# shangfuu/avse_challenge

Measured on AMD Instinct MI355X. Metric: utterances/sec (3s@16kHz + 75 lip frames), higher is better.
Workload: dtype fp32; 1 GPU; avse1 AV baseline train step (BASELINE configs[1]): HIP STFT front-end + AVNet (ResNet18 lip enc + TCN, dilated Conv2d audio net, LSTM fusion) fwd/bwd + Adam; global_batch=32, per_gpu_batch=32, seq_len=48000, stft_frames=376, lip_frames=75, lip_hw=96, parallelism=dp1, hip_graph=fwd+bwd+opt

## Files before the change

avse_challenge_amd/csrc/dconv.hip:

```cpp
#include <algorithm>

#include "bnact_cols.h"
#include "common.h"

namespace avse {
namespace dcf {

typedef _Float16 half8 __attribute__((ext_vector_type(8)));
typedef float floatx16 __attribute__((ext_vector_type(16)));
typedef int i4_t __attribute__((ext_vector_type(4)));
typedef __attribute__((address_space(3))) void lds_void_t;

constexpr int C = 64, KS = 5, NQ = 4, TP = 256, THREADS = 256, WAVES = THREADS / 64;
constexpr int ROWB = 64;
constexpr int WIMG = KS * C * ROWB;
constexpr int NSTG = KS * NQ;
constexpr int MAXD = 16;
constexpr int XIMG_MAX = (TP + 8 * MAXD) * ROWB;
constexpr int STAGE = XIMG_MAX + WIMG;
constexpr int NBUF = 3;
constexpr int MAXP = (XIMG_MAX + WIMG) / 1024 / WAVES + 1;
static_assert(NBUF * STAGE <= 160 * 1024, "LDS");

__device__ inline int swz(int r) { return (r >> 2) & 3; }

__device__ inline int split_exp(uint32_t mb) {
    const int ef = (int)((mb >> 23) & 0xff);
    if (mb == 0) return 0;
    const int k = ef == 0 ? -127 : ef - 127;
    return min(100, max(-100, 14 - k));
}

__device__ inline i4_t rsrc_of(const void* base, int64_t bytes) {
    if (bytes > 0x7FFFFFF0LL) bytes = 0x7FFFFFF0LL;
    const uint64_t a = (uint64_t)base;
    return i4_t{__builtin_amdgcn_readfirstlane((int)(uint32_t)a), __builtin_amdgcn_readfirstlane((int)((a >> 32) & 0xffff)),
                __builtin_amdgcn_readfirstlane((int)bytes), 0x00020000};
}

__device__ inline void dma16(i4_t r, uint32_t lds_addr, uint32_t voff) {
    asm volatile("s_mov_b32 m0, %2\n\tbuffer_load_dwordx4 %0, %1, 0 offen lds" ::"v"(voff), "s"(r), "s"(lds_addr)
                 : "memory");
}

__device__ inline uint32_t lds_u32(const void* p) {
    return __builtin_amdgcn_readfirstlane((uint32_t)(uintptr_t)(const lds_void_t*)p);
}

__device__ inline void wait_all_but(int n) {
    switch (n) {
        case 0: asm volatile("s_waitcnt vmcnt(0)" ::: "memory"); break;
        case 1: asm volatile("s_waitcnt vmcnt(1)" ::: "memory"); break;
        case 2: asm volatile("s_waitcnt vmcnt(2)" ::: "memory"); break;
        case 3: asm volatile("s_waitcnt vmcnt(3)" ::: "memory"); break;
        case 4: asm volatile("s_waitcnt vmcnt(4)" ::: "memory"); break;
        case 5: asm volatile("s_waitcnt vmcnt(5)" ::: "memory"); break;
        case 6: asm volatile("s_waitcnt vmcnt(6)" ::: "memory"); break;
        case 7: asm volatile("s_waitcnt vmcnt(7)" ::: "memory"); break;
        case 8: asm volatile("s_waitcnt vmcnt(8)" ::: "memory"); break;
        case 9: asm volatile("s_waitcnt vmcnt(9)" ::: "memory"); break;
        case 10: asm volatile("s_waitcnt vmcnt(10)" ::: "memory"); break;
        case 11: asm volatile("s_waitcnt vmcnt(11)" ::: "memory"); break;
        default: asm volatile("s_waitcnt vmcnt(12)" ::: "memory"); break;
    }
}

__device__ inline half8 frag(const uint8_t* img, int row, int c) {
    return *reinterpret_cast<const half8*>(img + row * ROWB + 16 * (c ^ swz(row)));
}

struct Args {
    const void* xq;
    const void* wq;
    const uint32_t* maxbits;
    const float* bias;
    float* y;
    int N, H, W, tiles;
    bnact::BnEpi bn;
};

template <int D, int NW, int WGS = 1, int EPI = 0>
__global__ __launch_bounds__(64 * NW, WGS) void fwd_kernel(Args a) {
    constexpr int TPX = 64 * NW, NSEG = NW == 4 ? 2 : 3;
    constexpr int NP = (TPX + 4 * D * NSEG + 15) / 16 * 16;
    constexpr int XIMG = NP * ROWB;
    constexpr int STG = XIMG + WIMG;
    constexpr int NB = WGS == 2 ? 2 : ((3 * STG <= 160 * 1024) ? 3 : 2);
    constexpr int PX = XIMG / 1024, PT = PX + WIMG / 1024;
    constexpr int MP = PT / NW + 1;
    __shared__ __attribute__((aligned(1024))) uint8_t lds[NB * STG];
    const int lane = threadIdx.x & 63;
    const int wave = __builtin_amdgcn_readfirstlane(threadIdx.x >> 6);
    const int bid = xcd_remap(blockIdx.x, gridDim.x);
    const int n = bid / a.tiles, t = bid % a.tiles;
    const int HW = a.H * a.W;
    const int p0 = t * TPX;
    const int r0 = p0 / a.W, w0 = p0 - r0 * a.W;
    const int n0 = min(TPX, a.W - w0), n1 = min(TPX - n0, a.W), n2 = TPX - n0 - n1;
    const int S1 = n0 + 4 * D, S2 = n0 + n1 + 8 * D;
    const i4_t rx = rsrc_of(a.xq, (int64_t)a.N * HW * 256);
    const i4_t rw = rsrc_of(a.wq, (int64_t)NSTG * WIMG);
    const uint32_t lds0 = lds_u32(lds);

    int pcol[MP], prow[MP];
    uint32_t pchunk[MP];
    const int npieces = (PT - wave + NW - 1) / NW;
#pragma unroll
    for (int m = 0; m < MP; ++m) {
        const int k = wave + NW * m;
        if (k < PX) {
            const int r = 16 * k + (lane >> 2), c = (lane & 3) ^ swz(r);
            int col, row;
            if (r < S1) {
                col = w0 - 2 * D + r;
                row = r0;
            } else if (r < S2 || NSEG == 2) {
                col = -2 * D + (r - S1);
                row = (n1 > 0 && r < S1 + n1 + 4 * D) ? r0 + 1 : -1000000;
            } else {
                col = -2 * D + (r - S2);
                row = (n2 > 0 && r < S2 + n2 + 4 * D) ? r0 + 2 : -1000000;
            }
            pcol[m] = (col >= 0 && col < a.W) ? col : -1;
            prow[m] = row;
            pchunk[m] = 16u * c;
        } else {
            const int r = 16 * (k - PX) + (lane >> 2), c = (lane & 3) ^ swz(r);
            pcol[m] = 0;
            prow[m] = 0;
            pchunk[m] = (uint32_t)(r * ROWB + 16 * c);
        }
    }
    auto issue = [&](int s) {
        const int kh = s / NQ, q = s % NQ;
        const uint32_t img = lds0 + (s % NB) * STG;
#pragma unroll
        for (int m = 0; m < MP; ++m) {
            if (m >= npieces) break;
            const int k = wave + NW * m;
            if (k < PX) {
                const int row = prow[m] + D * (kh - 2);
                const bool ok = pcol[m] >= 0 && row >= 0 && row < a.H;
                const uint32_t pix = ((uint32_t)n * (uint32_t)a.H + (uint32_t)row) * (uint32_t)a.W + (uint32_t)pcol[m];
                const uint32_t off = ok ? pix * 256u + (uint32_t)(q * 64) + pchunk[m] : 0x7FFFFFF0u;
                dma16(rx, img + k * 1024, off);
            } else {
                dma16(rw, img + XIMG + (k - PX) * 1024, (uint32_t)(s * WIMG) + pchunk[m]);
            }
        }
    };

    int posA[2];
#pragma unroll
    for (int i = 0; i < 2; ++i) {
        const int j = 64 * wave + 32 * i + (lane & 31);
        posA[i] = j + 4 * D * ((j >= n0) + (j >= n0 + n1));
    }
    const int hc = lane >> 5;

    floatx16 acc[2][2];
#pragma unroll
    for (int i = 0; i < 2; ++i)
#pragma unroll
        for (int j = 0; j < 2; ++j)
#pragma unroll
            for (int e = 0; e < 16; ++e) acc[i][j][e] = 0.f;

    issue(0);
    if (NB == 3) issue(1);
    for (int s = 0; s < NSTG; ++s) {
        if (NB == 3 && s + 1 < NSTG) wait_all_but(npieces);
        else asm volatile("s_waitcnt vmcnt(0)" ::: "memory");
        __builtin_amdgcn_s_barrier();
        asm volatile("" ::: "memory");
        if (s + NB - 1 < NSTG) issue(s + NB - 1);
        const uint8_t* ximg = lds + (s % NB) * STG;
        const uint8_t* wimg = ximg + XIMG;
#pragma unroll
        for (int kw = 0; kw < KS; ++kw) {
            half8 ah[2], al[2], bh[2], bl[2];
#pragma unroll
            for (int i = 0; i < 2; ++i) {
                const int r = posA[i] + D * kw;
                ah[i] = frag(ximg, r, hc);
                al[i] = frag(ximg, r, 2 + hc);
            }
#pragma unroll
            for (int j = 0; j < 2; ++j) {
                const int r = kw * C + 32 * j + (lane & 31);
                bh[j] = frag(wimg, r, hc);
                bl[j] = frag(wimg, r, 2 + hc);
            }
#pragma unroll
            for (int i = 0; i < 2; ++i)
#pragma unroll
                for (int j = 0; j < 2; ++j) {
                    acc[i][j] = __builtin_amdgcn_mfma_f32_32x32x16_f16(ah[i], bh[j], acc[i][j], 0, 0, 0);
                    acc[i][j] = __builtin_amdgcn_mfma_f32_32x32x16_f16(ah[i], bl[j], acc[i][j], 0, 0, 0);
                    acc[i][j] = __builtin_amdgcn_mfma_f32_32x32x16_f16(al[i], bh[j], acc[i][j], 0, 0, 0);
                }
        }
        if (NB == 2) {
            asm volatile("s_waitcnt lgkmcnt(0)" ::: "memory");
        }
    }

    const float scale = __builtin_ldexpf(1.f, -(split_exp(a.maxbits[0]) + split_exp(a.maxbits[1])));
    auto store = [&](int j) {
        const int o = 32 * j + (lane & 31);
        const float bv = a.bias ? a.bias[o] : 0.f;
#pragma unroll
        for (int i = 0; i < 2; ++i)
#pragma unroll
            for (int g = 0; g < 4; ++g)
#pragma unroll
                for (int e = 0; e < 4; ++e) {
                    const int p = p0 + 64 * wave + 32 * i + 8 * g + 4 * (lane >> 5) + e;
                    const float v = acc[i][j][4 * g + e] * scale + bv;
                    if constexpr (EPI != 0) acc[i][j][4 * g + e] = v;
                    if (p < HW) a.y[((int64_t)n * HW + p) * C + o] = v;
                }
    };
    if constexpr (EPI == 0) {
#pragma unroll
        for (int j = 0; j < 2; ++j) store(j);
    } else {
        constexpr int ENQ = EPI == 2 ? 4 : 3;
        float* part = reinterpret_cast<float*>(lds);
        __syncthreads();
        bnact::bn_epi_wave<bnact::ACT_RELU, EPI == 2>(
            a.bn, [&](int i, int j, int r) { return acc[i][j][r]; }, store, (int64_t)n * HW + p0 + 64 * wave,
            (int64_t)(n + 1) * HW, 0, C, lane, part + wave * ENQ * 64);
        __syncthreads();
        bnact::bn_epi_row<EPI == 2>(a.bn, part, NW, 1, (int64_t)bid, 0, C);
    }
}

constexpr int WG_CHUNK = 64;
constexpr int PIXB = 256;
constexpr int WTHREADS = 512, WWAVES = WTHREADS / 64;

typedef short s4_t __attribute__((ext_vector_type(4)));
typedef __attribute__((address_space(3))) s4_t lds_s4_t;

__device__ inline int tswz(int r, int c) { return c ^ (((r & 1) << 1) | ((r & 2) << 2)); }

__device__ inline half8 tfrag(const uint8_t* img, const int (&row)[2], int cb, int pl, int lane) {
    const int g = lane >> 4, i = lane & 15;
    const int q = 2 * cb + (g & 1);
    s4_t v[2];
#pragma unroll
    for (int u = 0; u < 2; ++u) {
        const int r = row[u];
        const int byte = q * 64 + pl * 32 + 8 * (i & 3);
        const int off = r * PIXB + 16 * tswz(r, byte >> 4) + (byte & 15);
        v[u] = __builtin_amdgcn_ds_read_tr16_b64_v4i16((lds_s4_t*)(img + off));
    }
    const s4_t w0 = v[0], w1 = v[1];
    const short __attribute__((ext_vector_type(8))) w = {w0[0], w0[1], w0[2], w0[3], w1[0], w1[1], w1[2], w1[3]};
    return __builtin_bit_cast(half8, w);
}

struct WArgs {
    const void* xq;
    const void* dyq;
    const uint32_t* xmax;
    const uint32_t* dymax;
    float* part;
    float* dbpart;
    int N, H, W, cpi, chunks, ranges;
};

struct ChunkPos {
    int n, p0, hA, wA0;
    __device__ void init(int c, int cpi, int W) {
        n = c / cpi;
        p0 = (c - n * cpi) * WG_CHUNK;
        hA = p0 / W;
        wA0 = p0 - hA * W;
    }
    __device__ void next(int HW, int W) {
        p0 += WG_CHUNK;
        if (p0 >= HW) {
            ++n;
            p0 = hA = wA0 = 0;
        } else {
            wA0 += WG_CHUNK;
            if (wA0 >= W) {
                wA0 -= W;
                ++hA;
            }
        }
    }
};

template <int D>
__global__ __launch_bounds__(WTHREADS, 1) void wgrad_kernel(WArgs a) {
    constexpr int NP = WG_CHUNK + 8 * D;
    constexpr int YIMG = WG_CHUNK * PIXB, XIMG = NP * PIXB, STG = YIMG + XIMG;
    constexpr int NB = (3 * STG <= 160 * 1024) ? 3 : 2;
    constexpr int PY = YIMG / 1024, PT = PY + XIMG / 1024;
    constexpr int MAXPW = PT / WWAVES + 1;
    __shared__ __attribute__((aligned(1024))) uint8_t lds[NB * STG];
    const int lane = threadIdx.x & 63;
    const int wave = __builtin_amdgcn_readfirstlane(threadIdx.x >> 6);
    const int bid = xcd_remap(blockIdx.x, gridDim.x);
    const int r = bid / KS, kh = bid % KS;
    const int c_lo = (int)((int64_t)r * a.chunks / a.ranges), c_hi = (int)((int64_t)(r + 1) * a.chunks / a.ranges);
    const int HW = a.H * a.W;
    const i4_t rx = rsrc_of(a.xq, (int64_t)a.N * HW * PIXB);
    const i4_t ry = rsrc_of(a.dyq, (int64_t)a.N * HW * PIXB);
    const uint32_t lds0 = lds_u32(lds);
    const int npieces = (PT - wave + WWAVES - 1) / WWAVES;
    const int pr = lane >> 4, pc = lane & 15;
    int pj[MAXPW];
    uint32_t psw[MAXPW];
#pragma unroll
    for (int m = 0; m < MAXPW; ++m) {
        const int k = wave + WWAVES * m;
        pj[m] = k < PY ? 4 * k + pr : 4 * (k - PY) + pr;
        psw[m] = 16u * tswz(pj[m], pc);
    }

    auto issue = [&](const ChunkPos& cp, int buf) {
        const int nA = min(WG_CHUNK, a.W - cp.wA0);
        const int row1 = cp.hA + D * (kh - 2), row2 = nA < WG_CHUNK ? row1 + 1 : -1000000;
        const int ybase = cp.n * HW + cp.p0;
        const int nHrow = cp.n * a.H;
        const uint32_t img = lds0 + buf * STG;
#pragma unroll
        for (int m = 0; m < MAXPW; ++m) {
            if (m >= npieces) break;
            const int k = wave + WWAVES * m;
            if (k < PY) {
                const int j = pj[m];
                const uint32_t off = cp.p0 + j < HW ? (uint32_t)(ybase + j) * PIXB + psw[m] : 0x7FFFFFF0u;
                dma16(ry, img + k * 1024, off);
            } else {
                const int q = pj[m];
                const bool s1 = q < nA + 4 * D;
                const int col = s1 ? cp.wA0 - 2 * D + q : q - nA - 6 * D;
                const int row = s1 ? row1 : row2;
                const bool ok = (unsigned)col < (unsigned)a.W && (unsigned)row < (unsigned)a.H;
                const uint32_t pix = (uint32_t)((nHrow + row) * a.W + col);
                dma16(rx, img + YIMG + (k - PY) * 1024, ok ? pix * PIXB + psw[m] : 0x7FFFFFF0u);
            }
        }
    };

    const int half = wave >> 2, ob = (wave >> 1) & 1, ib = wave & 1;
    const bool want_db = a.dbpart != nullptr && kh == 0 && ib == 0;
    floatx16 acc[KS], accb;
#pragma unroll
    for (int k = 0; k < KS; ++k)
#pragma unroll
        for (int e = 0; e < 16; ++e) acc[k][e] = 0.f;
#pragma unroll
    for (int e = 0; e < 16; ++e) accb[e] = 0.f;
    half8 ones;
#pragma unroll
    for (int e = 0; e < 8; ++e) ones[e] = (_Float16)1.0f;

    const int g = lane >> 4, li = lane & 15;
    ChunkPos cc, ci;
    cc.init(c_lo, a.cpi, a.W);
    ci = cc;
    if (c_lo < c_hi) {
        issue(ci, 0);
        ci.next(HW, a.W);
    }
    if (NB == 3 && c_lo + 1 < c_hi) {
        issue(ci, 1);
        ci.next(HW, a.W);
    }
    for (int c = c_lo; c < c_hi; ++c) {
        const int it = c - c_lo;
        const bool ahead = NB == 3 && c + 1 < c_hi;
        if (ahead) wait_all_but(npieces);
        else asm volatile("s_waitcnt vmcnt(0)" ::: "memory");
        __builtin_amdgcn_s_barrier();
        asm volatile("" ::: "memory");
        if (c + NB - 1 < c_hi) {
            issue(ci, (it + NB - 1) % NB);
            ci.next(HW, a.W);
        }
        const uint8_t* yimg = lds + (it % NB) * STG;
        const uint8_t* ximg = yimg + YIMG;
        const int nA = min(WG_CHUNK, a.W - cc.wA0);
#pragma unroll
        for (int s2 = 0; s2 < 2; ++s2) {
            const int s = 2 * half + s2;
            int ry_[2], rx_[2];
#pragma unroll
            for (int u = 0; u < 2; ++u) {
                const int j = 16 * s + 8 * (g >> 1) + (li >> 2) + 4 * u;
                ry_[u] = j;
                rx_[u] = j < nA ? j : j + 4 * D;
            }
            const half8 ah = tfrag(yimg, ry_, ob, 0, lane), al = tfrag(yimg, ry_, ob, 1, lane);
#pragma unroll
            for (int kw = 0; kw < KS; ++kw) {
                const int rk[2] = {rx_[0] + D * kw, rx_[1] + D * kw};
                const half8 bh = tfrag(ximg, rk, ib, 0, lane), bl = tfrag(ximg, rk, ib, 1, lane);
                acc[kw] = __builtin_amdgcn_mfma_f32_32x32x16_f16(ah, bh, acc[kw], 0, 0, 0);
                acc[kw] = __builtin_amdgcn_mfma_f32_32x32x16_f16(ah, bl, acc[kw], 0, 0, 0);
                acc[kw] = __builtin_amdgcn_mfma_f32_32x32x16_f16(al, bh, acc[kw], 0, 0, 0);
            }
            if (want_db) {
                accb = __builtin_amdgcn_mfma_f32_32x32x16_f16(ah, ones, accb, 0, 0, 0);
                accb = __builtin_amdgcn_mfma_f32_32x32x16_f16(al, ones, accb, 0, 0, 0);
            }
        }
        cc.next(HW, a.W);
    }
    const float sc = __builtin_ldexpf(1.f, -(split_exp(*a.xmax) + split_exp(*a.dymax)));
    float* pp = a.part + (((int64_t)r * 2 + half) * KS + kh) * KS * C * C;
#pragma unroll
    for (int kw = 0; kw < KS; ++kw)
#pragma unroll
        for (int q = 0; q < 4; ++q)
#pragma unroll
            for (int e = 0; e < 4; ++e) {
                const int o = 32 * ob + 8 * q + 4 * (lane >> 5) + e, i = 32 * ib + (lane & 31);
                pp[((int64_t)kw * C + o) * C + i] = acc[kw][4 * q + e] * sc;
            }
    if (want_db && (lane & 31) == 0) {
        const float sd = __builtin_ldexpf(1.f, -split_exp(*a.dymax));
#pragma unroll
        for (int q = 0; q < 4; ++q)
#pragma unroll
            for (int e = 0; e < 4; ++e)
                a.dbpart[((int64_t)r * 2 + half) * C + 32 * ob + 8 * q + 4 * (lane >> 5) + e] = accb[4 * q + e] * sd;
    }
}

__global__ void wgrad_reduce_kernel(const float* __restrict__ part, const float* __restrict__ dbpart, int slabs,
                                    float* __restrict__ dw, float* __restrict__ db) {
    constexpr int TOTAL = KS * KS * C * C;
    const int idx = blockIdx.x * blockDim.x + threadIdx.x;
    if (idx >= TOTAL) {
        if (db != nullptr && idx < TOTAL + C) {
            float v = 0.f;
            for (int g = 0; g < slabs; ++g) v += dbpart[(int64_t)g * C + idx - TOTAL];
            db[idx - TOTAL] = v;
        }
        return;
    }
    float v = 0.f;
    for (int g = 0; g < slabs; ++g) v += part[(int64_t)g * TOTAL + idx];
    const int i = idx % C, o = (idx / C) % C, kw = (idx / (C * C)) % KS, kh = idx / (KS * C * C);
    dw[((o * C + i) * KS + kh) * KS + kw] = v;
}

inline int wgrad_ranges(int chunks) { return std::max(1, std::min(chunks, 256 / KS * 1)); }

constexpr int AMAX_NT = 1024, AMAX_GRID = 256;
__global__ __launch_bounds__(AMAX_NT) void absmax_kernel(const float4* x, int64_t n4, uint32_t* out) {
    __shared__ uint32_t red[AMAX_NT / 64];
    float m = 0.f;
    const int64_t stride = (int64_t)gridDim.x * AMAX_NT;
    for (int64_t i0 = blockIdx.x * (int64_t)AMAX_NT + threadIdx.x; i0 < n4; i0 += 4 * stride) {
        float4 v[4];
#pragma unroll
        for (int u = 0; u < 4; ++u) v[u] = i0 + u * stride < n4 ? x[i0 + u * stride] : make_float4(0.f, 0.f, 0.f, 0.f);
#pragma unroll
        for (int u = 0; u < 4; ++u) m = fmaxf(m, fmaxf(fmaxf(fabsf(v[u].x), fabsf(v[u].y)), fmaxf(fabsf(v[u].z), fabsf(v[u].w))));
    }
    uint32_t b = __float_as_uint(m);
    for (int o = 32; o >= 1; o >>= 1) b = max(b, (uint32_t)__shfl_xor((int)b, o, 64));
    if ((threadIdx.x & 63) == 0) red[threadIdx.x >> 6] = b;
    __syncthreads();
    if (threadIdx.x == 0) {
        for (int k = 0; k < AMAX_NT / 64; ++k) b = max(b, red[k]);
        if (b) atomicMax(out, b);
    }
}

__device__ inline uint32_t split2(float x0, float x1, float sc, uint32_t& lo) {
    const float s0 = x0 * sc, s1 = x1 * sc;
    const _Float16 h0 = (_Float16)s0, h1 = (_Float16)s1;
    const _Float16 l0 = (_Float16)(s0 - (float)h0), l1 = (_Float16)(s1 - (float)h1);
    lo = (uint32_t)__builtin_bit_cast(uint16_t, l0) | ((uint32_t)__builtin_bit_cast(uint16_t, l1) << 16);
    return (uint32_t)__builtin_bit_cast(uint16_t, h0) | ((uint32_t)__builtin_bit_cast(uint16_t, h1) << 16);
}

__global__ void split_kernel(const float* x, int64_t nq, const uint32_t* maxbits, uint4* xq) {
    const float sc = __builtin_ldexpf(1.f, split_exp(maxbits[0]));
    for (int64_t i = blockIdx.x * (int64_t)blockDim.x + threadIdx.x; i < nq; i += (int64_t)gridDim.x * blockDim.x) {
        const float4* s = reinterpret_cast<const float4*>(x + i * 16);
        uint32_t hi[8], lo[8];
#pragma unroll
        for (int k = 0; k < 4; ++k) {
            const float4 v = s[k];
            hi[2 * k] = split2(v.x, v.y, sc, lo[2 * k]);
            hi[2 * k + 1] = split2(v.z, v.w, sc, lo[2 * k + 1]);
        }
        uint4* d = xq + i * 4;
        d[0] = uint4{hi[0], hi[1], hi[2], hi[3]};
        d[1] = uint4{hi[4], hi[5], hi[6], hi[7]};
        d[2] = uint4{lo[0], lo[1], lo[2], lo[3]};
        d[3] = uint4{lo[4], lo[5], lo[6], lo[7]};
    }
}

__global__ __launch_bounds__(1024) void wprep_kernel(const float* w, int transposed, uint32_t* maxbits, uint16_t* wq) {
    __shared__ uint32_t red[16];
    constexpr int TOT = C * C * KS * KS;
    float m = 0.f;
    for (int i = threadIdx.x; i < TOT; i += blockDim.x) m = fmaxf(m, fabsf(w[i]));
    uint32_t b = __float_as_uint(m);
    for (int o = 32; o >= 1; o >>= 1) b = max(b, (uint32_t)__shfl_xor((int)b, o, 64));
    if ((threadIdx.x & 63) == 0) red[threadIdx.x >> 6] = b;
    __syncthreads();
    b = 0;
    for (int k = 0; k < (int)(blockDim.x >> 6); ++k) b = max(b, red[k]);
    if (threadIdx.x == 0) maxbits[1] = b;
    const float sc = __builtin_ldexpf(1.f, split_exp(b));
    for (int e = threadIdx.x; e < TOT; e += blockDim.x) {
        const int c = e % 16, o = (e / 16) % C, kw = (e / (16 * C)) % KS, s = e / (16 * C * KS);
        const int kh = s / NQ, q = s % NQ, i = q * 16 + c;
        const float v = transposed ? w[((i * C + o) * KS + (KS - 1 - kh)) * KS + (KS - 1 - kw)]
                                   : w[((o * C + i) * KS + kh) * KS + kw];
        const float sv = v * sc;
        const _Float16 h = (_Float16)sv, l = (_Float16)(sv - (float)h);
        const int64_t row = ((int64_t)s * KS + kw) * C + o;
        wq[row * 32 + c] = __builtin_bit_cast(uint16_t, h);
        wq[row * 32 + 16 + c] = __builtin_bit_cast(uint16_t, l);
    }
}

__global__ __launch_bounds__(1024) void wprep2_kernel(const float* w, uint32_t* mb0, uint32_t* mb1, uint16_t* wq0,
                                                      uint16_t* wq1) {
    __shared__ uint32_t red[16];
    constexpr int TOT = C * C * KS * KS, PER = KS * C * 16;
    float m = 0.f;
    for (int i = threadIdx.x; i < TOT; i += 1024) m = fmaxf(m, fabsf(w[i]));
    uint32_t b = __float_as_uint(m);
    for (int o = 32; o >= 1; o >>= 1) b = max(b, (uint32_t)__shfl_xor((int)b, o, 64));
    if ((threadIdx.x & 63) == 0) red[threadIdx.x >> 6] = b;
    __syncthreads();
    b = 0;
    for (int k = 0; k < 16; ++k) b = max(b, red[k]);
    if (blockIdx.x == 0 && threadIdx.x == 0) {
        mb0[1] = b;
        if (mb1) mb1[1] = b;
    }
    const float sc = __builtin_ldexpf(1.f, split_exp(b));
    const int transposed = blockIdx.x / NSTG, s = blockIdx.x % NSTG;
    uint16_t* wq = transposed ? wq1 : wq0;
    const int kh = s / NQ, q = s % NQ;
    for (int e = threadIdx.x; e < PER; e += 1024) {
        const int c = e % 16, o = (e / 16) % C, kw = e / (16 * C);
        const int i = q * 16 + c;
        const float v = transposed ? w[((i * C + o) * KS + (KS - 1 - kh)) * KS + (KS - 1 - kw)]
                                   : w[((o * C + i) * KS + kh) * KS + kw];
        const float sv = v * sc;
        const _Float16 h = (_Float16)sv, l = (_Float16)(sv - (float)h);
        const int64_t row = ((int64_t)s * KS + kw) * C + o;
        wq[row * 32 + c] = __builtin_bit_cast(uint16_t, h);
        wq[row * 32 + 16 + c] = __builtin_bit_cast(uint16_t, l);
    }
}

}
}

using namespace avse::dcf;

extern "C" {

int64_t avse_dconv_wprep_bytes(void) { return (int64_t)NSTG * WIMG; }

int avse_split16(int64_t n_pix, const float* x, void* xq, uint32_t* maxbits, avse_stream_t stream) {
    if (!x || !xq || !maxbits) return AVSE_EINVAL;
    if (n_pix <= 0) return AVSE_ESHAPE;
    if (((uintptr_t)x & 15) || ((uintptr_t)xq & 15)) return AVSE_EALIGN;
    hipStream_t st = (hipStream_t)stream;
    if (hipMemsetAsync(maxbits, 0, 4, st) != hipSuccess) return AVSE_ELAUNCH;
    const int64_t n4 = n_pix * C / 4;
    hipLaunchKernelGGL(absmax_kernel, dim3((unsigned)std::max<int64_t>(1, std::min<int64_t>(AMAX_GRID, (n4 + AMAX_NT - 1) / AMAX_NT))),
                       dim3(AMAX_NT), 0, st, reinterpret_cast<const float4*>(x), n4, maxbits);
    AVSE_CHECK_LAUNCH();
    const int64_t nq = n_pix * NQ;
    const int blocks = (int)std::min<int64_t>((nq + 255) / 256, 8192);
    hipLaunchKernelGGL(split_kernel, dim3(blocks), dim3(256), 0, st, x, nq, maxbits, reinterpret_cast<uint4*>(xq));
    AVSE_CHECK_LAUNCH();
    return AVSE_OK;
}

int avse_split16_known(int64_t n_pix, const float* x, void* xq, const uint32_t* maxbits, avse_stream_t stream) {
    if (!x || !xq || !maxbits) return AVSE_EINVAL;
    if (n_pix <= 0) return AVSE_ESHAPE;
    if (((uintptr_t)x & 15) || ((uintptr_t)xq & 15)) return AVSE_EALIGN;
    const int64_t nq = n_pix * NQ;
    const int blocks = (int)std::min<int64_t>((nq + 255) / 256, 8192);
    hipLaunchKernelGGL(split_kernel, dim3(blocks), dim3(256), 0, (hipStream_t)stream, x, nq, maxbits,
                       reinterpret_cast<uint4*>(xq));
    AVSE_CHECK_LAUNCH();
    return AVSE_OK;
}

int avse_dconv_wprep(const float* w, int32_t transposed, void* wq, uint32_t* maxbits, avse_stream_t stream) {
    if (!w || !wq || !maxbits) return AVSE_EINVAL;
    hipLaunchKernelGGL(wprep_kernel, dim3(1), dim3(1024), 0, (hipStream_t)stream, w, transposed, maxbits,
                       reinterpret_cast<uint16_t*>(wq));
    AVSE_CHECK_LAUNCH();
    return AVSE_OK;
}

int avse_dconv_wprep2(const float* w, void* wq, void* wq_t, uint32_t* maxbits, uint32_t* maxbits_t,
                      avse_stream_t stream) {
    if (!w || !wq || !maxbits || (wq_t == nullptr) != (maxbits_t == nullptr)) return AVSE_EINVAL;
    hipLaunchKernelGGL(wprep2_kernel, dim3(wq_t ? 2 * NSTG : NSTG), dim3(1024), 0, (hipStream_t)stream, w, maxbits,
                       maxbits_t, reinterpret_cast<uint16_t*>(wq), reinterpret_cast<uint16_t*>(wq_t));
    AVSE_CHECK_LAUNCH();
    return AVSE_OK;
}

int64_t avse_dconv_wgrad16_workspace_bytes(int64_t N, int64_t H, int64_t W) {
    const int64_t chunks = N * ((H * W + WG_CHUNK - 1) / WG_CHUNK);
    return 4 * 2 * (int64_t)wgrad_ranges((int)std::min<int64_t>(chunks, 1 << 30)) * (KS * KS * C * C + C);
}

int avse_dconv_wgrad16(int64_t N, int64_t H, int64_t W, int64_t dil, const void* xq, const uint32_t* xmax,
                       const void* dyq, const uint32_t* dymax, float* dw, float* db, float* workspace,
                       avse_stream_t stream) {
    if (!xq || !xmax || !dyq || !dymax || !dw || !workspace) return AVSE_EINVAL;
    if (N <= 0 || H <= 0 || W < WG_CHUNK || (dil != 2 && dil != 4 && dil != 8 && dil != 16)) return AVSE_ESHAPE;
    if (N * H * W * 256 >= (1LL << 31) - 1024) return AVSE_ESHAPE;
    WArgs a;
    a.xq = xq;
    a.dyq = dyq;
    a.xmax = xmax;
    a.dymax = dymax;
    a.N = (int)N;
    a.H = (int)H;
    a.W = (int)W;
    a.cpi = (int)((H * W + WG_CHUNK - 1) / WG_CHUNK);
    a.chunks = (int)(N * a.cpi);
    a.ranges = wgrad_ranges(a.chunks);
    a.part = workspace;
    a.dbpart = db ? workspace + (int64_t)2 * a.ranges * KS * KS * C * C : nullptr;
    const dim3 grid((unsigned)(a.ranges * KS)), block(WTHREADS);
    hipStream_t st = (hipStream_t)stream;
    switch (dil) {
        case 2: hipLaunchKernelGGL(wgrad_kernel<2>, grid, block, 0, st, a); break;
        case 4: hipLaunchKernelGGL(wgrad_kernel<4>, grid, block, 0, st, a); break;
        case 8: hipLaunchKernelGGL(wgrad_kernel<8>, grid, block, 0, st, a); break;
        default: hipLaunchKernelGGL(wgrad_kernel<16>, grid, block, 0, st, a); break;
    }
    AVSE_CHECK_LAUNCH();
    constexpr int TOTAL = KS * KS * C * C;
    hipLaunchKernelGGL(wgrad_reduce_kernel, dim3((TOTAL + C + 255) / 256), dim3(256), 0, st, a.part, a.dbpart,
                       2 * a.ranges, dw, db);
    AVSE_CHECK_LAUNCH();
    return AVSE_OK;
}

static inline int dcf_nw(int64_t dil) { return dil <= 8 ? 4 : 8; }

int64_t avse_dconv_bn_rows(int64_t N, int64_t H, int64_t W, int64_t dil) {
    if (N <= 0 || H <= 0 || W < 256) return 0;
    return N * ((H * W + 64 * dcf_nw(dil) - 1) / (64 * dcf_nw(dil)));
}

static int dconv_launch(int64_t N, int64_t H, int64_t W, int64_t dil, const void* xq, const void* wq,
                        const uint32_t* maxbits, const float* bias, float* y, const avse::bnact::BnEpi* bn, int epi,
                        avse_stream_t stream);

int avse_dconv_fwd(int64_t N, int64_t H, int64_t W, int64_t dil, const void* xq, const void* wq,
                   const uint32_t* maxbits, const float* bias, float* y, avse_stream_t stream) {
    return dconv_launch(N, H, W, dil, xq, wq, maxbits, bias, y, nullptr, 0, stream);
}

int avse_dconv_dgrad_bn(int64_t N, int64_t H, int64_t W, int64_t dil, const void* dyq, const void* wq_t,
                        const uint32_t* maxbits, float* dx, const float* bn_x, const float* bn_stats,
                        const float* gamma, const float* beta, int32_t act, int32_t want_max, float* rows,
                        avse_stream_t stream) {
    if (!bn_x || !bn_stats || !rows) return AVSE_EINVAL;
    if (act != avse::bnact::ACT_RELU) return AVSE_ESHAPE;
    avse::bnact::BnEpi bn;
    bn.x = bn_x;
    bn.stats = bn_stats;
    bn.gamma = gamma;
    bn.beta = beta;
    bn.alpha = nullptr;
    bn.alpha_n = 0;
    bn.rows = rows;
    return dconv_launch(N, H, W, dil, dyq, wq_t, maxbits, nullptr, dx, &bn, want_max ? 2 : 1, stream);
}

static int dconv_launch(int64_t N, int64_t H, int64_t W, int64_t dil, const void* xq, const void* wq,
                        const uint32_t* maxbits, const float* bias, float* y, const avse::bnact::BnEpi* bn, int epi,
                        avse_stream_t stream) {
    if (!xq || !wq || !maxbits || !y) return AVSE_EINVAL;
    if (N <= 0 || H <= 0 || W < 256 || (dil != 2 && dil != 4 && dil != 8 && dil != 16)) return AVSE_ESHAPE;
    if (N * H * W * 256 >= (1LL << 31) - 1024) return AVSE_ESHAPE;
    Args a;
    a.xq = xq;
    a.wq = wq;
    a.maxbits = maxbits;
    a.bias = bias;
    a.y = y;
    a.N = (int)N;
    a.H = (int)H;
    a.W = (int)W;
    const int nw = dcf_nw(dil);
    if (bn) a.bn = *bn;
    else a.bn = avse::bnact::BnEpi{nullptr, nullptr, nullptr, nullptr, nullptr, 0, nullptr};
    a.tiles = (int)((H * W + 64 * nw - 1) / (64 * nw));
    const dim3 grid((unsigned)(N * a.tiles)), block(64 * nw);
    hipStream_t st = (hipStream_t)stream;
#define AVSE_DCF_CASES(E)                                                                           \
    switch (dil) {                                                                                  \
        case 2: hipLaunchKernelGGL((fwd_kernel<2, 4, 2, E>), grid, block, 0, st, a); break;         \
        case 4: hipLaunchKernelGGL((fwd_kernel<4, 4, 2, E>), grid, block, 0, st, a); break;         \
        case 8: hipLaunchKernelGGL((fwd_kernel<8, 4, 2, E>), grid, block, 0, st, a); break;         \
        default: hipLaunchKernelGGL((fwd_kernel<16, 8, 1, E>), grid, block, 0, st, a); break;       \
    }
    if (epi == 0) { AVSE_DCF_CASES(0) }
    else if (epi == 1) { AVSE_DCF_CASES(1) }
    else { AVSE_DCF_CASES(2) }
#undef AVSE_DCF_CASES
    AVSE_CHECK_LAUNCH();
    return AVSE_OK;
}

}
```

Measured before the change: 452.5 utt/s.

## Split weight-grad loop into LDS-load and MFMA phases with staggered wave halves

Restructures the dilated-conv weight-gradient main loop so each chunk first loads all A/B fragments from LDS into registers, then runs all MFMAs. The two wave halves are offset by one barrier segment, so one half does LDS reads while the other does MFMA work. Issue and wait points are reordered around sched_barriers to match. The aim is to overlap LDS read latency with matrix-core compute. In exchange it holds many more fragments in registers, which can cut occupancy, and the barrier choreography is fragile.

Measured after the change: 454.6 utt/s, median of 6. Within noise of the previous version (+0.5%).

```diff
diff --git a/avse_challenge_amd/csrc/dconv.hip b/avse_challenge_amd/csrc/dconv.hip
--- a/avse_challenge_amd/csrc/dconv.hip
+++ b/avse_challenge_amd/csrc/dconv.hip
@@ -362,29 +362,31 @@
     for (int e = 0; e < 8; ++e) ones[e] = (_Float16)1.0f;
 
     const int g = lane >> 4, li = lane & 15;
+    const int nch = c_hi - c_lo;
     ChunkPos cc, ci;
     cc.init(c_lo, a.cpi, a.W);
     ci = cc;
-    if (c_lo < c_hi) {
-        issue(ci, 0);
-        ci.next(HW, a.W);
-    }
-    if (NB == 3 && c_lo + 1 < c_hi) {
-        issue(ci, 1);
-        ci.next(HW, a.W);
-    }
-    for (int c = c_lo; c < c_hi; ++c) {
-        const int it = c - c_lo;
-        const bool ahead = NB == 3 && c + 1 < c_hi;
-        if (ahead) wait_all_but(npieces);
+    int ni = 0, islot = 0;
+    auto issue_next = [&]() {
+        if (ni < nch) {
+            issue(ci, islot);
+            ci.next(HW, a.W);
+            ++ni;
+            islot = islot + 1 == NB ? 0 : islot + 1;
+        }
+    };
+    auto wait_chunk = [&](int k) {
+        if (ni - 1 - k == 1) wait_all_but(npieces);
         else asm volatile("s_waitcnt vmcnt(0)" ::: "memory");
+    };
+    auto seg_barrier = [&]() {
+        __builtin_amdgcn_sched_barrier(0);
         __builtin_amdgcn_s_barrier();
-        asm volatile("" ::: "memory");
-        if (c + NB - 1 < c_hi) {
-            issue(ci, (it + NB - 1) % NB);
-            ci.next(HW, a.W);
-        }
-        const uint8_t* yimg = lds + (it % NB) * STG;
+        __builtin_amdgcn_sched_barrier(0);
+    };
+    half8 fa[2][2], fb[2][KS][2];
+    auto load = [&](int slot) {
+        const uint8_t* yimg = lds + slot * STG;
         const uint8_t* ximg = yimg + YIMG;
         const int nA = min(WG_CHUNK, a.W - cc.wA0);
 #pragma unroll
@@ -397,21 +399,52 @@
                 ry_[u] = j;
                 rx_[u] = j < nA ? j : j + 4 * D;
             }
-            const half8 ah = tfrag(yimg, ry_, ob, 0, lane), al = tfrag(yimg, ry_, ob, 1, lane);
+            fa[s2][0] = tfrag(yimg, ry_, ob, 0, lane);
+            fa[s2][1] = tfrag(yimg, ry_, ob, 1, lane);
 #pragma unroll
             for (int kw = 0; kw < KS; ++kw) {
                 const int rk[2] = {rx_[0] + D * kw, rx_[1] + D * kw};
-                const half8 bh = tfrag(ximg, rk, ib, 0, lane), bl = tfrag(ximg, rk, ib, 1, lane);
-                acc[kw] = __builtin_amdgcn_mfma_f32_32x32x16_f16(ah, bh, acc[kw], 0, 0, 0);
-                acc[kw] = __builtin_amdgcn_mfma_f32_32x32x16_f16(ah, bl, acc[kw], 0, 0, 0);
-                acc[kw] = __builtin_amdgcn_mfma_f32_32x32x16_f16(al, bh, acc[kw], 0, 0, 0);
-            }
+                fb[s2][kw][0] = tfrag(ximg, rk, ib, 0, lane);
+                fb[s2][kw][1] = tfrag(ximg, rk, ib, 1, lane);
+            }
+        }
+    };
+    auto compute = [&]() {
+#pragma unroll
+        for (int s2 = 0; s2 < 2; ++s2) {
+#pragma unroll
+            for (int pr = 0; pr < 3; ++pr)
+#pragma unroll
+                for (int kw = 0; kw < KS; ++kw)
+                    acc[kw] = __builtin_amdgcn_mfma_f32_32x32x16_f16(fa[s2][pr == 2], fb[s2][kw][pr == 1], acc[kw], 0, 0, 0);
             if (want_db) {
-                accb = __builtin_amdgcn_mfma_f32_32x32x16_f16(ah, ones, accb, 0, 0, 0);
-                accb = __builtin_amdgcn_mfma_f32_32x32x16_f16(al, ones, accb, 0, 0, 0);
-            }
-        }
+                accb = __builtin_amdgcn_mfma_f32_32x32x16_f16(fa[s2][0], ones, accb, 0, 0, 0);
+                accb = __builtin_amdgcn_mfma_f32_32x32x16_f16(fa[s2][1], ones, accb, 0, 0, 0);
+            }
+        }
+    };
+
+    issue_next();
+    if (NB == 3) issue_next();
+    wait_chunk(0);
+    seg_barrier();
+    if (half && nch > 0) {
+        if (NB == 2) issue_next();
+        seg_barrier();
+    }
+    int slot = 0;
+    for (int k = 0; k < nch; ++k) {
+        if (!half || NB == 3) issue_next();
+        load(slot);
         cc.next(HW, a.W);
+        slot = slot + 1 == NB ? 0 : slot + 1;
+        asm volatile("s_waitcnt lgkmcnt(0)" ::: "memory");
+        if (half) wait_chunk(k + 1);
+        seg_barrier();
+        if (half && NB == 2) issue_next();
+        compute();
+        if (!half) wait_chunk(k + 1);
+        if (!half || k + 1 < nch) seg_barrier();
     }
     const float sc = __builtin_ldexpf(1.f, -(split_exp(*a.xmax) + split_exp(*a.dymax)));
     float* pp = a.part + (((int64_t)r * 2 + half) * KS + kh) * KS * C * C;
```
